# mathwrx/Decouple-and-Couple_Learning_in_Multi-Modal_Brain_Tumor_Segmentation

Hardware: AMD Instinct MI355X
Metric: training volumes/sec (4x128^3) (higher is better)
Workload: dtype bf16x3 forward (split-bf16 MFMA operands hi.hi+hi.lo+lo.hi: logits within 1e-3 of the fp32 reference) / bf16 data-gradient / bf16 weight-gradient MFMA operands; f32 accumulate, f32 storage, f32 master weights; 1 GPU; configs[1]: 1xMI355X, batch 2 per GPU, 4-modality 128^3 synthetic BraTS patches; fwd + softmax_dice + 4 sub-region/edge losses + bwd + Adam(amsgrad); random-init weights, dropout on; global_batch=2, parallelism=dp1, precision=bf16x3, dgrad_precision=bf16, wgrad_precision=bf16, mode=plan

## Files before the change

decouple-and-couple_learning_in_multi-modal_brain_tumor_segmentation_amd/csrc/gemm.hip:

```cpp
#include "common.h"
#include <cstdlib>

typedef struct cwf_gemm_args GemmArgs;


template <int TM, int TN, int GK>
__global__ __launch_bounds__(256) void gemm_mfma_kernel(const GemmArgs a) {
  constexpr int LDA_S = GK + 1, LDB_S = TN + 16;
  constexpr int IM = TM / 32, JN = TN / 32;
  constexpr int SA = TM * GK / 256, SB = TN * GK / 256;
  __shared__ float As[TM * LDA_S];
  __shared__ float Bs[GK * LDB_S];
  const int tid = threadIdx.x, lane = tid & 63, wave = tid >> 6;
  const int wr = wave >> 1, wc = wave & 1;
  const int r = lane & 15, kq = lane >> 4;
  const int zb = blockIdx.z / a.ZH, zh = blockIdx.z % a.ZH;
  const int m0 = blockIdx.y * TM, n0 = blockIdx.x * TN;
  const int64_t a_zoff = zb * a.sa_zb + zh * a.sa_zh;
  const float* A = ((a.A2 && n0 >= a.split_n) ? a.A2 : a.A) + a_zoff;
  const bool tabB = a.B_tab[0] != nullptr;
  const float* B = tabB ? a.B_tab[blockIdx.z] : a.B + zb * a.sb_zb + zh * a.sb_zh;
  if (a.B2 && m0 >= a.split_m) B = a.B2 + zb * a.sb_zb + zh * a.sb_zh;
  const bool a_drop = a.a_drop_p > 0.f;
  float* rowsum = a.rowsum_tab[0] ? a.rowsum_tab[blockIdx.z] : a.rowsum;
  const bool do_rs = rowsum != nullptr && blockIdx.x == 0 && wc == 0;

  f32x4 acc[IM][JN], accr[IM];
#pragma unroll
  for (int i = 0; i < IM; ++i) {
    accr[i] = (f32x4){0.f, 0.f, 0.f, 0.f};
#pragma unroll
    for (int j = 0; j < JN; ++j) acc[i][j] = (f32x4){0.f, 0.f, 0.f, 0.f};
  }

  const bool a_kfast = (a.sa_k == 1);
  const bool b_nfast = (a.sb_n == 1);
  int am[SA], ak[SA], bk[SB], bn[SB];
#pragma unroll
  for (int i = 0; i < SA; ++i) {
    if (a_kfast) { ak[i] = tid % GK; am[i] = tid / GK + (256 / GK) * i; } else { am[i] = tid % TM; ak[i] = tid / TM + (256 / TM) * i; }
  }
#pragma unroll
  for (int i = 0; i < SB; ++i) {
    if (b_nfast) { bn[i] = tid % TN; bk[i] = tid / TN + (256 / TN) * i; } else { bk[i] = tid % GK; bn[i] = tid / GK + (256 / GK) * i; }
  }
  float ra[SA], rb[SB];
  auto fetch = [&](int k0) {
#pragma unroll
    for (int i = 0; i < SA; ++i) {
      const int gm = m0 + am[i], gk = k0 + ak[i];
      float v = 0.f;
      if (gm < a.M && gk < a.K) {
        const int64_t off = gm * a.sa_m + gk * a.sa_k;
        v = A[off];
        if (a_drop) v *= cwf_keep(a.rng, a.a_drop_off, (uint64_t)(a_zoff + off), a.a_drop_n, a.a_drop_p, a.a_drop_p2);
      }
      ra[i] = v;
    }
#pragma unroll
    for (int i = 0; i < SB; ++i) {
      const int gn = n0 + bn[i], gkb = k0 + bk[i];
      rb[i] = (gn < a.N && gkb < a.K) ? B[gkb * a.sb_k + gn * a.sb_n] : 0.f;
    }
  };
  fetch(0);
  for (int k0 = 0; k0 < a.K; k0 += GK) {
    if (k0) __syncthreads();
#pragma unroll
    for (int i = 0; i < SA; ++i) As[am[i] * LDA_S + ak[i]] = ra[i];
#pragma unroll
    for (int i = 0; i < SB; ++i) Bs[bk[i] * LDB_S + bn[i]] = rb[i];
    __syncthreads();
    if (k0 + GK < a.K) fetch(k0 + GK);
#pragma unroll
    for (int kk = 0; kk < GK / 4; ++kk) {
      float av[IM], bv[JN];
#pragma unroll
      for (int i = 0; i < IM; ++i) av[i] = As[(wr * (TM / 2) + i * 16 + r) * LDA_S + kk * 4 + kq];
#pragma unroll
      for (int j = 0; j < JN; ++j) bv[j] = Bs[(kk * 4 + kq) * LDB_S + wc * (TN / 2) + j * 16 + r];
#pragma unroll
      for (int i = 0; i < IM; ++i)
#pragma unroll
        for (int j = 0; j < JN; ++j) acc[i][j] = __builtin_amdgcn_mfma_f32_16x16x4f32(av[i], bv[j], acc[i][j], 0, 0, 0);
      if (do_rs) {
#pragma unroll
        for (int i = 0; i < IM; ++i) accr[i] = __builtin_amdgcn_mfma_f32_16x16x4f32(av[i], 1.0f, accr[i], 0, 0, 0);
      }
    }
  }
  const int64_t c_zoff = zb * a.sc_zb + zh * a.sc_zh;
  float* C = a.C_tab[0] ? a.C_tab[blockIdx.z] : a.C + c_zoff;
  float* C2 = a.C2 ? a.C2 + c_zoff : nullptr;
  const float* bias = a.bias_tab[0] ? a.bias_tab[blockIdx.z] : a.bias;
  const float* R = a.residual ? a.residual + zb * a.sr_zb + zh * a.sr_zh : nullptr;
  const bool c_drop = a.c_drop_p > 0.f;
#pragma unroll
  for (int i = 0; i < IM; ++i)
#pragma unroll
    for (int j = 0; j < JN; ++j) {
      const int gn = n0 + wc * (TN / 2) + j * 16 + r;
      if (gn >= a.N) continue;
      const float bv = bias ? bias[gn] : 0.f;
#pragma unroll
      for (int e = 0; e < 4; ++e) {
        const int gm = m0 + wr * (TM / 2) + i * 16 + kq * 4 + e;
        if (gm >= a.M) continue;
        const int64_t off = gm * a.sc_m + gn;
        float v = acc[i][j][e] * a.alpha + bv;
        if (C2) C2[off] = v;
        if (a.act == 1) v = 0.5f * v * (1.f + erff(v * 0.70710678118654752440f));
        if (c_drop) v *= cwf_keep(a.rng, a.c_drop_off, (uint64_t)(c_zoff + off), a.c_drop_n, a.c_drop_p, a.c_drop_p2);
        if (R) v += R[gm * a.sr_m + gn];
        float* p = C + off;
        if (a.accumulate) v += *p;
        *p = v;
      }
    }
  if (do_rs && r == 0) {
#pragma unroll
    for (int i = 0; i < IM; ++i)
#pragma unroll
      for (int e = 0; e < 4; ++e) {
        const int gm = m0 + wr * (TM / 2) + i * 16 + kq * 4 + e;
        if (gm < a.M) rowsum[gm] = (a.rowsum_acc ? rowsum[gm] : 0.f) + accr[i][e];
      }
  }
}

template <int TM, int TN, int GK, bool AK, bool BN>
__global__ __launch_bounds__(256) void gemm_mfma_v_kernel(const GemmArgs a) {
  constexpr int LDA_S = GK + 1, LDB_S = TN + 16;
  constexpr int IM = TM / 32, JN = TN / 32;
  constexpr int SA = TM * GK / 1024, SB = TN * GK / 1024;
  __shared__ float As[TM * LDA_S];
  __shared__ __attribute__((aligned(16))) float Bs[GK * LDB_S];
  const int tid = threadIdx.x, lane = tid & 63, wave = tid >> 6;
  const int wr = wave >> 1, wc = wave & 1;
  const int r = lane & 15, kq = lane >> 4;
  const int zb = blockIdx.z / a.ZH, zh = blockIdx.z % a.ZH;
  const int m0 = blockIdx.y * TM, n0 = blockIdx.x * TN;
  const int64_t a_zoff = zb * a.sa_zb + zh * a.sa_zh;
  const float* A = ((a.A2 && n0 >= a.split_n) ? a.A2 : a.A) + a_zoff;
  const bool tabB = a.B_tab[0] != nullptr;
  const float* B = tabB ? a.B_tab[blockIdx.z] : a.B + zb * a.sb_zb + zh * a.sb_zh;
  if (a.B2 && m0 >= a.split_m) B = a.B2 + zb * a.sb_zb + zh * a.sb_zh;
  const bool a_drop = a.a_drop_p > 0.f;
  float* rowsum = a.rowsum_tab[0] ? a.rowsum_tab[blockIdx.z] : a.rowsum;
  const bool do_rs = rowsum != nullptr && blockIdx.x == 0 && wc == 0;

  f32x4 acc[IM][JN], accr[IM];
#pragma unroll
  for (int i = 0; i < IM; ++i) {
    accr[i] = (f32x4){0.f, 0.f, 0.f, 0.f};
#pragma unroll
    for (int j = 0; j < JN; ++j) acc[i][j] = (f32x4){0.f, 0.f, 0.f, 0.f};
  }
  int am[SA], ak[SA], bk[SB], bn[SB];
#pragma unroll
  for (int i = 0; i < SA; ++i) {
    if (AK) { ak[i] = (tid % (GK / 4)) * 4; am[i] = tid / (GK / 4) + (1024 / GK) * i; }
    else { am[i] = (tid % (TM / 4)) * 4; ak[i] = tid / (TM / 4) + (1024 / TM) * i; }
  }
#pragma unroll
  for (int i = 0; i < SB; ++i) {
    if (BN) { bn[i] = (tid % (TN / 4)) * 4; bk[i] = tid / (TN / 4) + (1024 / TN) * i; }
    else { bk[i] = (tid % (GK / 4)) * 4; bn[i] = tid / (GK / 4) + (1024 / GK) * i; }
  }
  f32x4 ra[SA], rb[SB];
  auto fetch = [&](int k0) {
#pragma unroll
    for (int i = 0; i < SA; ++i) {
      const int gm = m0 + am[i], gk = k0 + ak[i];
      f32x4 v = {0.f, 0.f, 0.f, 0.f};
      if (gm < a.M && gk < a.K) {
        const int64_t off = gm * a.sa_m + gk * a.sa_k;
        v = *reinterpret_cast<const f32x4*>(A + off);
        if (a_drop) {
          const int64_t st = AK ? 1 : a.sa_m;
#pragma unroll
          for (int c = 0; c < 4; ++c) v[c] *= cwf_keep(a.rng, a.a_drop_off, (uint64_t)(a_zoff + off + c * st), a.a_drop_n, a.a_drop_p, a.a_drop_p2);
        }
      }
      ra[i] = v;
    }
#pragma unroll
    for (int i = 0; i < SB; ++i) {
      const int gn = n0 + bn[i], gkb = k0 + bk[i];
      rb[i] = (gn < a.N && gkb < a.K) ? *reinterpret_cast<const f32x4*>(B + gkb * a.sb_k + gn * a.sb_n) : (f32x4){0.f, 0.f, 0.f, 0.f};
    }
  };
  fetch(0);
  for (int k0 = 0; k0 < a.K; k0 += GK) {
    if (k0) __syncthreads();
#pragma unroll
    for (int i = 0; i < SA; ++i)
#pragma unroll
      for (int c = 0; c < 4; ++c) {
        if (AK) As[am[i] * LDA_S + ak[i] + c] = ra[i][c];
        else As[(am[i] + c) * LDA_S + ak[i]] = ra[i][c];
      }
#pragma unroll
    for (int i = 0; i < SB; ++i) {
      if (BN) *reinterpret_cast<f32x4*>(&Bs[bk[i] * LDB_S + bn[i]]) = rb[i];
      else {
#pragma unroll
        for (int c = 0; c < 4; ++c) Bs[(bk[i] + c) * LDB_S + bn[i]] = rb[i][c];
      }
    }
    __syncthreads();
    if (k0 + GK < a.K) fetch(k0 + GK);
#pragma unroll
    for (int kk = 0; kk < GK / 4; ++kk) {
      float av[IM], bv[JN];
#pragma unroll
      for (int i = 0; i < IM; ++i) av[i] = As[(wr * (TM / 2) + i * 16 + r) * LDA_S + kk * 4 + kq];
#pragma unroll
      for (int j = 0; j < JN; ++j) bv[j] = Bs[(kk * 4 + kq) * LDB_S + wc * (TN / 2) + j * 16 + r];
#pragma unroll
      for (int i = 0; i < IM; ++i)
#pragma unroll
        for (int j = 0; j < JN; ++j) acc[i][j] = __builtin_amdgcn_mfma_f32_16x16x4f32(av[i], bv[j], acc[i][j], 0, 0, 0);
      if (do_rs) {
#pragma unroll
        for (int i = 0; i < IM; ++i) accr[i] = __builtin_amdgcn_mfma_f32_16x16x4f32(av[i], 1.0f, accr[i], 0, 0, 0);
      }
    }
  }
  const int64_t c_zoff = zb * a.sc_zb + zh * a.sc_zh;
  float* C = a.C_tab[0] ? a.C_tab[blockIdx.z] : a.C + c_zoff;
  float* C2 = a.C2 ? a.C2 + c_zoff : nullptr;
  const float* bias = a.bias_tab[0] ? a.bias_tab[blockIdx.z] : a.bias;
  const float* R = a.residual ? a.residual + zb * a.sr_zb + zh * a.sr_zh : nullptr;
  const bool c_drop = a.c_drop_p > 0.f;
#pragma unroll
  for (int i = 0; i < IM; ++i)
#pragma unroll
    for (int j = 0; j < JN; ++j) {
      const int gn = n0 + wc * (TN / 2) + j * 16 + r;
      if (gn >= a.N) continue;
      const float bv = bias ? bias[gn] : 0.f;
#pragma unroll
      for (int e = 0; e < 4; ++e) {
        const int gm = m0 + wr * (TM / 2) + i * 16 + kq * 4 + e;
        if (gm >= a.M) continue;
        const int64_t off = gm * a.sc_m + gn;
        float v = acc[i][j][e] * a.alpha + bv;
        if (C2) C2[off] = v;
        if (a.act == 1) v = 0.5f * v * (1.f + erff(v * 0.70710678118654752440f));
        if (c_drop) v *= cwf_keep(a.rng, a.c_drop_off, (uint64_t)(c_zoff + off), a.c_drop_n, a.c_drop_p, a.c_drop_p2);
        if (R) v += R[gm * a.sr_m + gn];
        float* p = C + off;
        if (a.accumulate) v += *p;
        *p = v;
      }
    }
  if (do_rs && r == 0) {
#pragma unroll
    for (int i = 0; i < IM; ++i)
#pragma unroll
      for (int e = 0; e < 4; ++e) {
        const int gm = m0 + wr * (TM / 2) + i * 16 + kq * 4 + e;
        if (gm < a.M) rowsum[gm] = (a.rowsum_acc ? rowsum[gm] : 0.f) + accr[i][e];
      }
  }
}

static bool gemm_vec_ok(const GemmArgs& a, bool* ak, bool* bn) {
  auto al = [](const void* p) { return (reinterpret_cast<uintptr_t>(p) & 15) == 0; };
  auto m4 = [](int64_t v) { return (v & 3) == 0; };
  if (!m4(a.sa_zb) || !m4(a.sa_zh) || !m4(a.sb_zb) || !m4(a.sb_zh)) return false;
  if (!al(a.A) || (a.A2 && !al(a.A2)) || (a.B && !al(a.B)) || (a.B2 && !al(a.B2))) return false;
  for (int z = 0; z < 4; ++z)
    if (a.B_tab[z] && !al(a.B_tab[z])) return false;
  if (a.sa_k == 1 && m4(a.K) && m4(a.sa_m)) *ak = true;
  else if (a.sa_m == 1 && m4(a.M) && m4(a.sa_k)) *ak = false;
  else return false;
  if (a.sb_n == 1 && m4(a.N) && m4(a.sb_k)) *bn = true;
  else if (a.sb_k == 1 && m4(a.K) && m4(a.sb_n)) *bn = false;
  else return false;
  if (a.B2 && (a.split_m & 3)) return false;
  return true;
}

struct GemmVariant { bool vec; int tm; bool ak, bn; };
static GemmVariant gemm_variant(const GemmArgs& a) {
  const int64_t wg64 = (int64_t)cdiv(a.N, 64) * cdiv(a.M, 64) * a.ZB * a.ZH;
  GemmVariant v = {false, wg64 >= 256 ? 64 : 32, false, false};
  if (a.K >= 64 && gemm_vec_ok(a, &v.ak, &v.bn)) v.vec = true;
  else v.ak = v.bn = false;
  return v;
}

static int gemm_check(const GemmArgs& a) {
  if (!a.A || (!a.B && !a.B_tab[0]) || (!a.C && !a.C_tab[0]) || a.M <= 0 || a.N <= 0 || a.K <= 0 || a.ZB <= 0 || a.ZH <= 0) return CWF_E_BADARG;
  if ((a.B_tab[0] || a.bias_tab[0] || a.C_tab[0] || a.rowsum_tab[0]) && (a.ZH != 1 || a.ZB > 4)) return CWF_E_BADARG;
  if ((int64_t)a.ZB * a.ZH > 65535) return CWF_E_TOOLARGE;
  if ((a.A2 && (a.split_n & 63)) || (a.B2 && (a.split_m & 63))) return CWF_E_BADARG;
  if ((a.a_drop_p > 0.f || a.c_drop_p > 0.f) && !a.rng) return CWF_E_BADARG;
  if (a.rowsum && (int64_t)a.ZB * a.ZH != 1) return CWF_E_BADARG;
  for (int z = 0; z < a.ZB && z < 4; ++z)
    if ((a.B_tab[0] && !a.B_tab[z]) || (a.bias_tab[0] && !a.bias_tab[z]) || (a.C_tab[0] && !a.C_tab[z]) || (a.rowsum_tab[0] && !a.rowsum_tab[z])) return CWF_E_BADARG;
  return 0;
}

extern "C" int cwf_gemm_ex(const struct cwf_gemm_args* args, void* stream) {
  if (!args) return CWF_E_BADARG;
  const GemmArgs& a = *args;
  const int rc = gemm_check(a);
  if (rc) return rc;
  const GemmVariant v = gemm_variant(a);
  const bool big = v.tm == 64;
  if (v.vec) {
    dim3 grid(cdiv(a.N, big ? 64 : 32), cdiv(a.M, big ? 64 : 32), a.ZB * a.ZH);
#define CWF_GV(AKv, BNv) do { if (big) hipLaunchKernelGGL((gemm_mfma_v_kernel<64, 64, 32, AKv, BNv>), grid, dim3(256), 0, cwf_stream(stream), a); \
                              else hipLaunchKernelGGL((gemm_mfma_v_kernel<32, 32, 64, AKv, BNv>), grid, dim3(256), 0, cwf_stream(stream), a); } while (0)
    if (v.ak && v.bn) CWF_GV(true, true); else if (v.ak) CWF_GV(true, false); else if (v.bn) CWF_GV(false, true); else CWF_GV(false, false);
#undef CWF_GV
    CWF_LAUNCH_CHECK();
    return 0;
  }
  if (big) {
    dim3 grid(cdiv(a.N, 64), cdiv(a.M, 64), a.ZB * a.ZH);
    hipLaunchKernelGGL((gemm_mfma_kernel<64, 64, 32>), grid, dim3(256), 0, cwf_stream(stream), a);
  } else {
    dim3 grid(cdiv(a.N, 32), cdiv(a.M, 32), a.ZB * a.ZH);
    hipLaunchKernelGGL((gemm_mfma_kernel<32, 32, 32>), grid, dim3(256), 0, cwf_stream(stream), a);
  }
  CWF_LAUNCH_CHECK();
  return 0;
}

extern "C" int cwf_debug_gemm_variant(const struct cwf_gemm_args* args, int* out) {
  if (!args || !out) return CWF_E_BADARG;
  const int rc = gemm_check(*args);
  if (rc) return rc;
  const GemmVariant v = gemm_variant(*args);
  out[0] = v.vec; out[1] = v.tm; out[2] = v.ak; out[3] = v.bn;
  return 0;
}

extern "C" int cwf_gemm(const float* A, int64_t sa_m, int64_t sa_k, int64_t sa_zb, int64_t sa_zh,
                        const float* B, int64_t sb_k, int64_t sb_n, int64_t sb_zb, int64_t sb_zh,
                        float* C, int64_t sc_m, int64_t sc_zb, int64_t sc_zh,
                        const float* bias, const float* residual, int64_t sr_m, int64_t sr_zb, int64_t sr_zh,
                        int M, int Nn, int K, int ZB, int ZH, float alpha, int act, int accumulate, void* stream) {
  GemmArgs a = {};
  a.A = A; a.sa_m = sa_m; a.sa_k = sa_k; a.sa_zb = sa_zb; a.sa_zh = sa_zh;
  a.B = B; a.sb_k = sb_k; a.sb_n = sb_n; a.sb_zb = sb_zb; a.sb_zh = sb_zh;
  a.C = C; a.sc_m = sc_m; a.sc_zb = sc_zb; a.sc_zh = sc_zh;
  a.bias = bias; a.residual = residual; a.sr_m = sr_m; a.sr_zb = sr_zb; a.sr_zh = sr_zh;
  a.M = M; a.N = Nn; a.K = K; a.ZB = ZB; a.ZH = ZH; a.alpha = alpha; a.act = act; a.accumulate = accumulate;
  return cwf_gemm_ex(&a, stream);
}

template <int PER>
__global__ __launch_bounds__(256) void layernorm_fwd_kernel(const float* __restrict__ x, const float* __restrict__ gamma, const float* __restrict__ beta,
                                                           float* __restrict__ y, float* __restrict__ mean, float* __restrict__ rstd, int rows, int E, float eps) {
  const int row = blockIdx.x * 4 + (threadIdx.x >> 6), lane = threadIdx.x & 63;
  if (row >= rows) return;
  const float* xr = x + (int64_t)row * E;
  float v[PER]; float s = 0.f;
#pragma unroll
  for (int i = 0; i < PER; ++i) { v[i] = xr[lane + 64 * i]; s += v[i]; }
  const float mu = wave_sum(s) / (float)E;
// ... 377 lines not shown
```

decouple-and-couple_learning_in_multi-modal_brain_tumor_segmentation_amd/cwf/_lib.py:

```python
from __future__ import annotations

import ctypes as C
import os

_HERE = os.path.dirname(os.path.abspath(__file__))
LIB_PATH = os.path.join(_HERE, "libcwf_hip.so")

P = C.c_void_p
I = C.c_int
L = C.c_int64
F = C.c_float
U = C.c_uint32
U64 = C.c_uint64
D = C.c_double

SIGNATURES = {
    "cwf_version": [],
    "cwf_conv": [P, P],
    "cwf_conv_x16_ok": [I, I, I, I, I, I, I],
    "cwf_debug_wsd": [I],
    "cwf_debug_wsd_launches": [],
    "cwf_wgrad": [P, P, P],
    "cwf_gather_split_bf16": [P, I, L, P],
    "cwf_wgrad_nsplit": [I, I, I, I, I, I, I],
    "cwf_wgrad_partial_floats": [I, I, I, I, I, I, I],
    "cwf_wgrad_slab_floats": [I, I, I],
    "cwf_wgrad_reduce": [P, I, L, P, P, P, P],
    "cwf_gather_batched": [P, I, L, P],
    "cwf_in_finalize": [P, P, P, I, L, F, P],
    "cwf_in_stats": [P, I, P, I, L, I, P],
    "cwf_norm_act_add": [P, I, P, P, F, P, I, P, I, I, L, I, P],
    "cwf_in_bwd_stats": [P, I, P, I, P, P, F, P, I, L, I, P],
    "cwf_in_bwd_apply": [P, I, P, I, P, P, F, P, P, I, P, I, I, L, I, P],
    "cwf_in_bwd_apply_ex": [P, I, P, I, P, P, F, P, P, I, P, I, P, P, I, L, I, P],
    "cwf_norm_act_add_ex": [P, I, P, P, F, P, I, P, I, P, I, L, I, P],
    "cwf_to_bf16": [P, I, P, P, F, P, I, L, I, P],
    "cwf_gemm": [P, L, L, L, L, P, L, L, L, L, P, L, L, L, P, P, L, L, L, I, I, I, I, I, F, I, I, P],
    "cwf_layernorm_fwd": [P, P, P, P, P, P, I, I, F, P],
    "cwf_layernorm_bwd": [P, P, P, P, P, P, P, P, I, I, I, P],
    "cwf_softmax_rows": [P, L, I, I, P],
    "cwf_softmax_rows_bwd": [P, P, L, I, I, P],
    "cwf_gelu_bwd": [P, P, P, L, P],
    "cwf_colsum": [P, L, I, I, P, I, P],
    "cwf_window_to_tokens": [P, I, P, I, I, I, I, I, I, I, I, P],
    "cwf_tokens_to_window": [P, P, I, I, I, I, I, I, I, I, I, I, P],
    "cwf_token_scores": [P, P, L, P, I, I, I, P],
    "cwf_topk": [P, P, I, I, I, P],
    "cwf_gather_tokens": [P, P, P, L, P, F, P, I, I, I, I, P],
    "cwf_gather_tokens_bwd": [P, P, P, P, P, L, I, I, I, I, P],
    "cwf_scatter_rows": [P, P, P, L, L, P, L, P, I, I, I, I, P],
    "cwf_scatter_rows_bwd": [P, P, P, P, L, P, I, P, L, L, P, L, I, I, I, I, P],
    "cwf_upsample_softmax": [P, I, P, I, I, I, I, I, I, P],
    "cwf_upsample_softmax_bwd": [P, P, P, I, I, I, I, I, I, I, P, P],
    "cwf_channel_softmax": [P, I, P, L, I, P],
    "cwf_channel_softmax_bwd": [P, P, P, I, L, I, P],
    "cwf_dice_ce_sums": [P, P, U, P, I, L, I, P],
    "cwf_dice_ce_finalize": [P, P, P, I, L, I, P],
    "cwf_dice_ce_bwd": [P, P, U, P, P, P, I, L, I, P],
    "cwf_adam_amsgrad": [P, I, L, C.c_double, C.c_double, C.c_double, C.c_double, C.c_double, I, I, P, P],
    "cwf_adam_amsgrad_scaled": [P, I, L, C.c_double, C.c_double, C.c_double, C.c_double, C.c_double, I, I, P, F, P],
    "cwf_grad_add": [P, P, P, L, P],
    "cwf_grad_norm_clip": [P, L, F, F, P, P, P],
    "cwf_adam_amsgrad_ex": [P, I, L, C.c_double, C.c_double, C.c_double, C.c_double, C.c_double, I, I, P, F, P, P, F, P],
    "cwf_optim_step": [I, P, I, L, C.c_double, C.c_double, P, C.c_double, C.c_double, C.c_double, I, I, P, C.c_double, C.c_double, I, I,
                       F, P, P, F, P],
    "cwf_wgrad_reduce_batched": [P, I, P],
    "cwf_dropout_mask": [P, L, F, F, C.c_uint64, C.c_uint64, P],
    "cwf_mul": [P, P, P, L, P],
    "cwf_add": [P, P, P, L, P],
    "cwf_channel_scale": [P, I, P, P, I, I, L, I, P],
    "cwf_copy_strided": [P, I, P, I, L, I, P],
    "cwf_add3": [P, P, P, P, L, P],
    "cwf_bcast3": [P, P, L, P],
    "cwf_stats_channel_sum": [P, P, I, I, P],
    "cwf_gemm_ex": [P, P],
    "cwf_attn_fwd": [P, L, P, L, I, I, I, I, F, P, U64, F, P],
    "cwf_attn_bwd": [P, L, P, L, P, I, I, I, I, F, P, U64, F, P],
    "cwf_ln_pair_fwd": [P, P, I, P, P, P, P, P, P, P, I, I, F, P],
    "cwf_ln_pair_bwd": [P, P, P, P, P, I, P, P, P, P, P, P, P, P, P, I, I, I, P],
    "cwf_gelu_bwd_drop": [P, P, P, L, P, U64, F, P],
    "cwf_token_scores2": [P, P, L, P, L, P, P, I, I, I, P],
    "cwf_topk_inv": [P, P, P, P, P, P, I, I, I, P],
    "cwf_index_inv": [P, P, I, I, I, P],
    "cwf_gather_multi": [P, I, I, I, I, F, P, F, P],
    "cwf_scatter_inv": [P, P, P, L, L, P, L, P, P, I, I, I, P],
    "cwf_scatter_bwd": [P, P, P, P, P, P, L, L, P, L, P, L, P, L, L, P, L, I, I, I, I, P],
    "cwf_token_grad": [P, P, P, L, P, P, P, L, P, L, P, U64, U64, F, P, I, I, I, I, P],
    "cwf_head_grad": [P, P, P, P, L, P, P, I, I, P],
    "cwf_dice_ce_finalize_multi": [P, P, P, P, I, I, L, I, P],
    "cwf_head_loss_sums": [P, I, I, P, P, P, I, I, I, I, I, P],
    "cwf_head_loss_bwd": [P, I, I, P, P, P, P, P, I, P, I, I, I, I, I, P],
    "cwf_head_loss_bwd_ex": [P, I, I, P, P, P, P, P, I, I, P, I, I, I, I, I, P],
    "cwf_ln_pair_fwd_g": [P, P, I, P, I, P, P, P, I, I, F, P],
    "cwf_ln_pair_bwd_g": [P, P, P, P, P, I, P, I, P, P, P, I, I, I, P],
    "cwf_token_scores2_g": [P, P, P, I, I, P, P, I, I, I, P],
    "cwf_head_grad_g": [P, P, P, P, L, P, P, I, I, I, P],
    "cwf_window_to_tokens_g": [P, I, P, I, I, I, I, I, I, I, I, I, P],
    "cwf_tokens_to_window_g": [P, P, I, I, I, I, I, I, I, I, I, I, P],
    "cwf_cat3_channels": [P, P, P, P, L, I, P],
    "cwf_stitch_windows": [P, P, I, P],
    "cwf_argmax_dice": [P, L, L, L, P, P, P, I, L, P],
    "cwf_argmax_metrics": [P, L, L, L, P, P, P, I, L, P],
    "cwf_region_bits": [P, P, L, P],
    "cwf_hausdorff_workspace": [I, I, I, I, I],
    "cwf_hausdorff": [P, P, I, I, I, I, I, D, D, D, I, I, P, P, P, P, L, P],
    "cwf_surface_metrics_workspace": [I, I, I, I, I],
    "cwf_surface_metrics": [P, P, I, I, I, I, I, D, D, D, I, I, P, I, P, P, P, P, P, P, P, P, L, P],
    "cwf_signed_distance_workspace": [I, I, I, I, I],
    "cwf_signed_distance": [P, P, P, I, I, I, I, I, P, P],
    "cwf_boundary_sums": [P, P, P, P, I, I, L, I, P],
    "cwf_boundary_finalize": [P, P, P, P, I, I, L, P],
    "cwf_boundary_bwd": [P, P, P, P, P, I, I, L, I, P],
    "cwf_topk_ce_workspace": [I, L],
    "cwf_topk_ce": [P, P, U, L, P, P, P, I, L, I, P, P],
    "cwf_topk_ce_bwd": [P, P, U, P, P, P, I, L, I, P],
    "cwf_focal_workspace": [I, L, I],
    "cwf_focal_loss": [P, P, P, I, P, P, P, P, I, L, I, P, P],
    "cwf_focal_loss_bwd": [P, P, P, I, P, P, P, P, I, L, I, P],
    "cwf_lovasz_workspace": [I, L, I],
    "cwf_lovasz": [P, P, P, I, I, P, P, P, P, I, L, P, P],
    "cwf_lovasz_bwd": [P, P, I, P, P, P, I, L, P],
    "cwf_components_workspace": [I, I, I, I, I],
    "cwf_components": [P, I, I, I, I, I, I, P, P, P, P, P, L, P],
    "cwf_postprocess_labels": [P, P, P, P, P, I, I, I, I, I, I, I, I, I, I, I, I, P, P, P],
    "cwf_label_metrics": [P, P, P, L, P],
    "cwf_dilate_bits": [P, P, I, I, I, I, I, I, P, L, P],
    "cwf_lesionwise_workspace": [I, I, I, I, I],
    "cwf_lesionwise": [P, P, I, I, I, I, I, I, L, D, P, P, P, P, P, P, L, P],
# ... 108 lines not shown


class PrepElasticSample(C.Structure):
    _fields_ = PrepAffineSample._fields_ + [("disp", P), ("G0", I), ("G1", I), ("G2", I)]


class IntensitySample(C.Structure):
    _fields_ = [("taps", (F * 7) * 4), ("amp", F * 4), ("key", U64), ("gamma", F * 4), ("blur", I), ("noise", I), ("gam", I)]


class FocalParams(C.Structure):
    _fields_ = [("fn", D), ("fp", D), ("exponent", D), ("smooth", D), ("gamma", D), ("ce_ratio", D), ("class_weight", D * 4)]


INTENSITY_TILE = (10, 10, 32)


def intensity_ws_floats(nb, crop):
    tiles = 1
    for c, t in zip(crop, INTENSITY_TILE):
        tiles *= (int(c) + t - 1) // t
    return 8 * int(nb) * tiles


class AcquireSample(C.Structure):
    _fields_ = [("bias", P * 4), ("G0", I), ("G1", I), ("G2", I), ("bias_mask", I), ("contrast_mask", I), ("lowres_mask", I),
                ("factor", F * 4), ("lattice", (I * 3) * 4)]


ACQUIRE_TILE = (32, 8, 32)


def acquire_ws_doubles(nb, crop):
    tiles = 1
    for c, t in zip(crop, ACQUIRE_TILE):
        tiles *= (int(c) + t - 1) // t
    return 12 * int(nb) * tiles


WINDOW_MAX_STARTS = 128


class WindowGrid(C.Structure):
    _fields_ = [("B", I), ("S", I * 3), ("r", I * 3), ("n", I * 3), ("start", (I * WINDOW_MAX_STARTS) * 3)]


class WindowBox(C.Structure):
    _fields_ = [("full", I * 3), ("lo", I * 3)]


NORM_WS_DOUBLES = 2568
GRADNORM_WS_DOUBLES = 1024
RULE_ADAMW, RULE_SGD = 1, 2
RESTYPE_INT64 = {"cwf_debug_wsd_launches", "cwf_wgrad_partial_floats", "cwf_wgrad_slab_floats", "cwf_hausdorff_workspace", "cwf_components_workspace",
                 "cwf_lesionwise_workspace", "cwf_surface_metrics_workspace", "cwf_lesionwise_ex_workspace", "cwf_signed_distance_workspace",
                 "cwf_topk_ce_workspace", "cwf_focal_workspace", "cwf_lovasz_workspace", "cwf_class_locations_workspace", "cwf_nonzero_box_workspace"}
LOCATIONS_TILE = 16384
NONZERO_BOX_TILE = 4096

_lib = None


class CwfError(RuntimeError):
    pass


def load():
    global _lib
    if _lib is not None:
        return _lib
    if not os.path.exists(LIB_PATH):
        raise CwfError("libcwf_hip.so is not built (%s); run `python __graft_entry__.py` or `make -C csrc`. "
                       "There is no CPU fallback." % LIB_PATH)
    lib = C.CDLL(LIB_PATH)
    for name, args in SIGNATURES.items():
        fn = getattr(lib, name)
        fn.argtypes = args
        fn.restype = L if name in RESTYPE_INT64 else I
    lib.cwf_arch.restype = C.c_char_p
    lib.cwf_arch.argtypes = []
    lib.cwf_plan_last_error.restype = C.c_char_p
    lib.cwf_plan_last_error.argtypes = []
    _lib = lib
    return lib


def check(rc, name):
    if rc != 0:
        raise CwfError("%s failed with status %d" % (name, rc))
```

include/cwf_hip.h:

```cpp
#ifndef CWF_HIP_H
#define CWF_HIP_H
#include <stdint.h>
#ifdef __cplusplus
extern "C" {
#endif

#define CWF_E_BADARG   (-1)
#define CWF_E_TOOLARGE (-2)
#define CWF_E_ALIGN    (-3)

int cwf_version(void);
const char* cwf_arch(void);

enum { CWF_CONV3_S1 = 0, CWF_CONV3_S2 = 1, CWF_CONV1 = 2, CWF_CONVT2 = 3, CWF_CONV3_S2_DGRAD = 4, CWF_CONVT2_DGRAD = 5 };
enum { CWF_FP32 = 0, CWF_BF16X3 = 1, CWF_BF16 = 2 };

struct cwf_conv_args {
  int op, precision;
  const float* x; int x_ldc; const void* wpk; const float* bias; float* y; int y_ldc;
  const float* in_scale; const float* in_shift; float in_slope;
  const float* residual; int r_ldc; const float* out_scale; double* stats;
  const float* nb_x; int nb_ldc; const float* nb_scale; const float* nb_shift; float nb_slope;
  const void* x16; const void* zero16; void* y16;
  const float* w_raw;
// ... 17 lines not shown
  int groups; const float* x_g[3]; const float* dy_g[3]; float* partial_g[3];
  int N, Di, Hi, Wi, Cin, Do, Ho, Wo, Cout;
};
int cwf_wgrad(const struct cwf_wgrad_args* args , int* nsplit_used , void* stream);
int cwf_wgrad_reduce(const float* partial, int nsplit, int64_t slab_floats,
                     const int32_t* inv_map, float* dW, float* db, void* stream);
struct cwf_wgrad_reduce_desc { const float* partial; const int32_t* inv; float* dW; float* db; int64_t slab; int32_t nsplit; int32_t pad_; };
int cwf_wgrad_reduce_batched(const struct cwf_wgrad_reduce_desc* table, int nlayers, void* stream);

struct cwf_gather_desc { const float* src; float* dst; const int32_t* map; int64_t n; };

int cwf_gather_split_bf16(const struct cwf_gather_desc* table, int nlayers, int64_t max_n, void* stream);

int cwf_gather_batched(const struct cwf_gather_desc* table, int nlayers, int64_t max_n, void* stream);

int cwf_in_finalize(const double* stats, float* scale, float* shift, int NC, int64_t V, float eps, void* stream);
int cwf_in_stats(const float* x, int x_ldc, double* stats, int N, int64_t V, int C, void* stream);
int cwf_norm_act_add(const float* x, int x_ldc, const float* scale, const float* shift, float slope,
                     const float* residual, int r_ldc, float* y, int y_ldc, int N, int64_t V, int C, void* stream);
int cwf_in_bwd_stats(const float* dy, int dy_ldc, const float* x, int x_ldc, const float* scale, const float* shift,
                     float slope, double* sums, int N, int64_t V, int C, void* stream);
int cwf_in_bwd_apply(const float* dy, int dy_ldc, const float* x, int x_ldc, const float* scale, const float* shift,
                     float slope, const double* sums, const float* dx_add, int a_ldc, float* dx, int dx_ldc,
                     int N, int64_t V, int C, void* stream);

int cwf_in_bwd_apply_ex(const float* dy, int dy_ldc, const float* x, int x_ldc, const float* scale, const float* shift,
                        float slope, const double* sums, const float* dx_add, int a_ldc, float* dx, int dx_ldc,
                        void* dx16, void* xa16, int N, int64_t V, int C, void* stream);
int cwf_norm_act_add_ex(const float* x, int x_ldc, const float* scale, const float* shift, float slope,
                        const float* residual, int r_ldc, float* y, int y_ldc, void* y16, int N, int64_t V, int C, void* stream);
int cwf_to_bf16(const float* x, int x_ldc, const float* scale, const float* shift, float slope, void* y16,
                int N, int64_t V, int C, void* stream);
int cwf_gemm(const float* A, int64_t sa_m, int64_t sa_k, int64_t sa_zb, int64_t sa_zh,
             const float* B, int64_t sb_k, int64_t sb_n, int64_t sb_zb, int64_t sb_zh,
             float* C, int64_t sc_m, int64_t sc_zb, int64_t sc_zh,
             const float* bias, const float* residual, int64_t sr_m, int64_t sr_zb, int64_t sr_zh,
             int M, int Nn, int K, int ZB, int ZH, float alpha, int act, int accumulate, void* stream);
struct cwf_gemm_args {
  const float* A; int64_t sa_m, sa_k, sa_zb, sa_zh;
  const float* B; int64_t sb_k, sb_n, sb_zb, sb_zh;
  float* C; int64_t sc_m, sc_zb, sc_zh;
  const float* bias; const float* residual; int64_t sr_m, sr_zb, sr_zh;
  int M, N, K, ZB, ZH; float alpha; int act; int accumulate;
  const float* A2; int split_n;
  const float* B2; int split_m;
  float* C2;
  float* rowsum; int rowsum_acc;
  const uint64_t* rng;
  uint64_t a_drop_off, a_drop_n; float a_drop_p, a_drop_p2;
  uint64_t c_drop_off, c_drop_n; float c_drop_p, c_drop_p2;
  const float* B_tab[4]; const float* bias_tab[4]; float* C_tab[4]; float* rowsum_tab[4];
};
int cwf_gemm_ex(const struct cwf_gemm_args* args , void* stream);

int cwf_attn_fwd(const float* qkv, int64_t ld, float* o, int64_t ldo, int Z, int T, int E, int heads, float scale,
                 const uint64_t* rng, uint64_t drop_off, float drop_p, void* stream);
int cwf_attn_bwd(const float* qkv, int64_t ld, const float* d_o, int64_t ldo, float* dqkv, int Z, int T, int E, int heads,
                 float scale, const uint64_t* rng, uint64_t drop_off, float drop_p, void* stream);

int cwf_ln_pair_fwd(const float* x, const float* x2, int perm_T, const float* g1, const float* b1, const float* g2, const float* b2,
                    float* ya, float* yb, float* stats, int rows, int E, float eps, void* stream);
struct cwf_ln_group_params { const float* g1[4]; const float* b1[4]; const float* g2[4]; const float* b2[4];
                             float* dg1[4]; float* db1[4]; float* dg2[4]; float* db2[4]; };
int cwf_ln_pair_fwd_g(const float* x, const float* x2, int perm_T, const struct cwf_ln_group_params* h_params, int groups,
                      float* ya, float* yb, float* stats, int rows, int E, float eps, void* stream);
int cwf_ln_pair_bwd_g(const float* dy, const float* da, const float* db, const float* x, const float* x2, int perm_T,
                      const struct cwf_ln_group_params* h_params, int groups, const float* stats, float* dx, float* dx2,
                      int rows, int E, int accumulate_params, void* stream);
int cwf_ln_pair_bwd(const float* dy, const float* da, const float* db, const float* x, const float* x2, int perm_T,
                    const float* g1, const float* g2, const float* stats, float* dx, float* dx2,
                    float* dg1, float* db1, float* dg2, float* db2, int rows, int E, int accumulate_params, void* stream);
int cwf_gelu_bwd_drop(const float* z, const float* dh, float* dz, int64_t n, const uint64_t* rng, uint64_t off, float p, void* stream);

int cwf_layernorm_fwd(const float* x, const float* gamma, const float* beta, float* y, float* mean, float* rstd,
                      int rows, int E, float eps, void* stream);
int cwf_layernorm_bwd(const float* dy, const float* x, const float* gamma, const float* mean, const float* rstd,
                      float* dx, float* dgamma, float* dbeta, int rows, int E, int accumulate, void* stream);
int cwf_softmax_rows(float* s, int64_t rows, int cols, int ld, void* stream);
int cwf_softmax_rows_bwd(const float* p, float* dp_inout, int64_t rows, int cols, int ld, void* stream);
int cwf_gelu_bwd(const float* x, const float* dy, float* dx, int64_t n, void* stream);
int cwf_colsum(const float* x, int64_t rows, int cols, int ld, float* out, int accumulate, void* stream);

int cwf_window_to_tokens(const float* x, int x_ldc, float* tok, int B, int D, int H, int W, int C,
                         int p0, int p1, int p2, void* stream);
int cwf_tokens_to_window(const float* tok, float* x, int x_ldc, int B, int D, int H, int W, int C,
                         int p0, int p1, int p2, int accumulate, void* stream);
int cwf_token_scores(const float* feats, const float* query, int64_t query_bstride, float* score,
                     int B, int T, int E, void* stream);
int cwf_topk(const float* score, int32_t* index, int B, int T, int k, void* stream);
int cwf_gather_tokens(const float* feats, const int32_t* index, const float* head, int64_t head_bstride,
                      const float* keep, float pe_odd, float* seq, int B, int T, int k, int E, void* stream);
int cwf_gather_tokens_bwd(const float* dseq, const int32_t* index, const float* keep, float* dfeats, float* dhead,
                          int64_t dhead_bstride, int B, int T, int k, int E, void* stream);
int cwf_scatter_rows(const float* feats, const int32_t* index, const float* rows, int64_t rows_ld, int64_t rows_bs,
                     const float* gate, int64_t gate_bs, float* out, int B, int T, int k, int E, void* stream);
int cwf_scatter_rows_bwd(const float* dout, const int32_t* index, const float* scat, const float* gate, int64_t gate_bs,
                         float* dfeats, int accumulate, float* drows, int64_t drows_ld, int64_t drows_bs,
                         float* dgate, int64_t dgate_bs, int B, int T, int k, int E, void* stream);

int cwf_token_scores2(const float* feats, const float* q1, int64_t q1_bstride, const float* q2, int64_t q2_bstride,
                      float* s1, float* s2, int B, int T, int E, void* stream);
int cwf_token_scores2_g(const float* feats, const float* const* h_q1, const float* const* h_q2, int groups, int group_B,
                        float* s1, float* s2, int B, int T, int E, void* stream);
int cwf_topk_inv(const float* score0, int32_t* index0, int32_t* inv0, const float* score1, int32_t* index1, int32_t* inv1,
                 int B, int T, int k, void* stream);
int cwf_index_inv(const int32_t* index, int32_t* inv, int B, int T, int k, void* stream);
// ... 262 lines not shown
```

Baseline: 117.9 volumes/s.

## Add compile-time-K panel GEMM kernel with deep register prefetch for common shapes

Adds a GEMM kernel specialised on a compile-time K. It prefetches several k-panels into registers ahead of use (depth D) and fully unrolls the panel loop. It also XOR-swizzles the shared-memory layout for the non-N-contiguous B operand. A routing table sends vectorisable GEMMs with matching K and tile size to this kernel by default, aiming to hide global-load latency and cut LDS bank conflicts in the transformer-path GEMMs. The shared epilogue is factored into a helper. The cost is more register pressure and code size from the deep prefetch and full unroll, plus extra template instantiations.

```diff
diff --git a/decouple-and-couple_learning_in_multi-modal_brain_tumor_segmentation_amd/csrc/gemm.hip b/decouple-and-couple_learning_in_multi-modal_brain_tumor_segmentation_amd/csrc/gemm.hip
--- a/decouple-and-couple_learning_in_multi-modal_brain_tumor_segmentation_amd/csrc/gemm.hip
+++ b/decouple-and-couple_learning_in_multi-modal_brain_tumor_segmentation_amd/csrc/gemm.hip
@@ -1,7 +1,51 @@
 #include "common.h"
 #include <cstdlib>
+#include <type_traits>
 
 typedef struct cwf_gemm_args GemmArgs;
+
+template <int TM, int TN>
+__device__ __forceinline__ void gemm_epilogue(const GemmArgs& a, const f32x4 (&acc)[TM / 32][TN / 32], const f32x4 (&accr)[TM / 32], int zb, int zh,
+                                              int m0, int n0, int wr, int wc, int r, int kq, bool do_rs, float* rowsum) {
+  constexpr int IM = TM / 32, JN = TN / 32;
+  const int64_t c_zoff = zb * a.sc_zb + zh * a.sc_zh;
+  float* C = a.C_tab[0] ? a.C_tab[blockIdx.z] : a.C + c_zoff;
+  float* C2 = a.C2 ? a.C2 + c_zoff : nullptr;
+  const float* bias = a.bias_tab[0] ? a.bias_tab[blockIdx.z] : a.bias;
+  const float* R = a.residual ? a.residual + zb * a.sr_zb + zh * a.sr_zh : nullptr;
+  const bool c_drop = a.c_drop_p > 0.f;
+#pragma unroll
+  for (int i = 0; i < IM; ++i)
+#pragma unroll
+    for (int j = 0; j < JN; ++j) {
+      const int gn = n0 + wc * (TN / 2) + j * 16 + r;
+      if (gn >= a.N) continue;
+      const float bv = bias ? bias[gn] : 0.f;
+#pragma unroll
+      for (int e = 0; e < 4; ++e) {
+        const int gm = m0 + wr * (TM / 2) + i * 16 + kq * 4 + e;
+        if (gm >= a.M) continue;
+        const int64_t off = gm * a.sc_m + gn;
+        float v = acc[i][j][e] * a.alpha + bv;
+        if (C2) C2[off] = v;
+        if (a.act == 1) v = 0.5f * v * (1.f + erff(v * 0.70710678118654752440f));
+        if (c_drop) v *= cwf_keep(a.rng, a.c_drop_off, (uint64_t)(c_zoff + off), a.c_drop_n, a.c_drop_p, a.c_drop_p2);
+        if (R) v += R[gm * a.sr_m + gn];
+        float* p = C + off;
+        if (a.accumulate) v += *p;
+        *p = v;
+      }
+    }
+  if (do_rs && r == 0) {
+#pragma unroll
+    for (int i = 0; i < IM; ++i)
+#pragma unroll
+      for (int e = 0; e < 4; ++e) {
+        const int gm = m0 + wr * (TM / 2) + i * 16 + kq * 4 + e;
+        if (gm < a.M) rowsum[gm] = (a.rowsum_acc ? rowsum[gm] : 0.f) + accr[i][e];
+      }
+  }
+}
 
 
 template <int TM, int TN, int GK>
@@ -89,43 +133,7 @@
       }
     }
   }
-  const int64_t c_zoff = zb * a.sc_zb + zh * a.sc_zh;
-  float* C = a.C_tab[0] ? a.C_tab[blockIdx.z] : a.C + c_zoff;
-  float* C2 = a.C2 ? a.C2 + c_zoff : nullptr;
-  const float* bias = a.bias_tab[0] ? a.bias_tab[blockIdx.z] : a.bias;
-  const float* R = a.residual ? a.residual + zb * a.sr_zb + zh * a.sr_zh : nullptr;
-  const bool c_drop = a.c_drop_p > 0.f;
-#pragma unroll
-  for (int i = 0; i < IM; ++i)
-#pragma unroll
-    for (int j = 0; j < JN; ++j) {
-      const int gn = n0 + wc * (TN / 2) + j * 16 + r;
-      if (gn >= a.N) continue;
-      const float bv = bias ? bias[gn] : 0.f;
-#pragma unroll
-      for (int e = 0; e < 4; ++e) {
-        const int gm = m0 + wr * (TM / 2) + i * 16 + kq * 4 + e;
-        if (gm >= a.M) continue;
-        const int64_t off = gm * a.sc_m + gn;
-        float v = acc[i][j][e] * a.alpha + bv;
-        if (C2) C2[off] = v;
-        if (a.act == 1) v = 0.5f * v * (1.f + erff(v * 0.70710678118654752440f));
-        if (c_drop) v *= cwf_keep(a.rng, a.c_drop_off, (uint64_t)(c_zoff + off), a.c_drop_n, a.c_drop_p, a.c_drop_p2);
-        if (R) v += R[gm * a.sr_m + gn];
-        float* p = C + off;
-        if (a.accumulate) v += *p;
-        *p = v;
-      }
-    }
-  if (do_rs && r == 0) {
-#pragma unroll
-    for (int i = 0; i < IM; ++i)
-#pragma unroll
-      for (int e = 0; e < 4; ++e) {
-        const int gm = m0 + wr * (TM / 2) + i * 16 + kq * 4 + e;
-        if (gm < a.M) rowsum[gm] = (a.rowsum_acc ? rowsum[gm] : 0.f) + accr[i][e];
-      }
-  }
+  gemm_epilogue<TM, TN>(a, acc, accr, zb, zh, m0, n0, wr, wc, r, kq, do_rs, rowsum);
 }
 
 template <int TM, int TN, int GK, bool AK, bool BN>
@@ -227,43 +235,149 @@
       }
     }
   }
-  const int64_t c_zoff = zb * a.sc_zb + zh * a.sc_zh;
-  float* C = a.C_tab[0] ? a.C_tab[blockIdx.z] : a.C + c_zoff;
-  float* C2 = a.C2 ? a.C2 + c_zoff : nullptr;
-  const float* bias = a.bias_tab[0] ? a.bias_tab[blockIdx.z] : a.bias;
-  const float* R = a.residual ? a.residual + zb * a.sr_zb + zh * a.sr_zh : nullptr;
-  const bool c_drop = a.c_drop_p > 0.f;
-#pragma unroll
-  for (int i = 0; i < IM; ++i)
-#pragma unroll
-    for (int j = 0; j < JN; ++j) {
-      const int gn = n0 + wc * (TN / 2) + j * 16 + r;
-      if (gn >= a.N) continue;
-      const float bv = bias ? bias[gn] : 0.f;
-#pragma unroll
-      for (int e = 0; e < 4; ++e) {
-        const int gm = m0 + wr * (TM / 2) + i * 16 + kq * 4 + e;
-        if (gm >= a.M) continue;
-        const int64_t off = gm * a.sc_m + gn;
-        float v = acc[i][j][e] * a.alpha + bv;
-        if (C2) C2[off] = v;
-        if (a.act == 1) v = 0.5f * v * (1.f + erff(v * 0.70710678118654752440f));
-        if (c_drop) v *= cwf_keep(a.rng, a.c_drop_off, (uint64_t)(c_zoff + off), a.c_drop_n, a.c_drop_p, a.c_drop_p2);
-        if (R) v += R[gm * a.sr_m + gn];
-        float* p = C + off;
-        if (a.accumulate) v += *p;
-        *p = v;
-      }
-    }
-  if (do_rs && r == 0) {
-#pragma unroll
-    for (int i = 0; i < IM; ++i)
-#pragma unroll
-      for (int e = 0; e < 4; ++e) {
-        const int gm = m0 + wr * (TM / 2) + i * 16 + kq * 4 + e;
-        if (gm < a.M) rowsum[gm] = (a.rowsum_acc ? rowsum[gm] : 0.f) + accr[i][e];
-      }
-  }
+  gemm_epilogue<TM, TN>(a, acc, accr, zb, zh, m0, n0, wr, wc, r, kq, do_rs, rowsum);
+}
+
+template <int TM, int TN, int PK, int KC, int D, bool AK, bool BN>
+__global__ __launch_bounds__(256) void gemm_mfma_p_kernel(const GemmArgs a) {
+  constexpr int NP = (KC + PK - 1) / PK;
+  constexpr int K4 = (KC + 3) / 4 * 4;
+  constexpr int LDA_S = PK + 1, LDB_S = TN + 16;
+  constexpr int IM = TM / 32, JN = TN / 32;
+  constexpr int SA = TM * PK / 1024, SB = TN * PK / 1024;
+  static_assert(D >= 2 && PK % 4 == 0 && SA >= 1 && SB >= 1, "panel geometry");
+  static_assert(KC % 4 == 0 || (!AK && BN), "an operand with 16-byte loads along k needs K % 4 == 0");
+  __shared__ float As[TM * LDA_S];
+  __shared__ __attribute__((aligned(16))) float Bs[PK * LDB_S];
+  const int tid = threadIdx.x, lane = tid & 63, wave = tid >> 6;
+  const int wr = wave >> 1, wc = wave & 1;
+  const int r = lane & 15, kq = lane >> 4;
+  const int zb = blockIdx.z / a.ZH, zh = blockIdx.z % a.ZH;
+  const int m0 = blockIdx.y * TM, n0 = blockIdx.x * TN;
+  const int64_t a_zoff = zb * a.sa_zb + zh * a.sa_zh;
+  const float* A = ((a.A2 && n0 >= a.split_n) ? a.A2 : a.A) + a_zoff;
+  const bool tabB = a.B_tab[0] != nullptr;
+  const float* B = tabB ? a.B_tab[blockIdx.z] : a.B + zb * a.sb_zb + zh * a.sb_zh;
+  if (a.B2 && m0 >= a.split_m) B = a.B2 + zb * a.sb_zb + zh * a.sb_zh;
+  const bool a_drop = a.a_drop_p > 0.f;
+  float* rowsum = a.rowsum_tab[0] ? a.rowsum_tab[blockIdx.z] : a.rowsum;
+  const bool do_rs = rowsum != nullptr && blockIdx.x == 0 && wc == 0;
+
+  f32x4 acc[IM][JN], accr[IM];
+#pragma unroll
+  for (int i = 0; i < IM; ++i) {
+    accr[i] = (f32x4){0.f, 0.f, 0.f, 0.f};
+#pragma unroll
+    for (int j = 0; j < JN; ++j) acc[i][j] = (f32x4){0.f, 0.f, 0.f, 0.f};
+  }
+  int am[SA], ak[SA], bk[SB], bn[SB];
+  int64_t aoff[SA], boff[SB];
+  bool a_ok[SA], b_ok[SB];
+  const int64_t a_sk = AK ? 1 : a.sa_k, a_sm = AK ? a.sa_m : 1, b_sn = BN ? 1 : a.sb_n, b_sk = BN ? a.sb_k : 1;
+#pragma unroll
+  for (int i = 0; i < SA; ++i) {
+    if (AK) { ak[i] = (tid % (PK / 4)) * 4; am[i] = tid / (PK / 4) + (1024 / PK) * i; }
+    else { am[i] = (tid % (TM / 4)) * 4; ak[i] = tid / (TM / 4) + (1024 / TM) * i; }
+    const int gm = m0 + am[i];
+    a_ok[i] = gm < a.M;
+    aoff[i] = min(gm, a.M - (AK ? 1 : 4)) * a_sm;
+  }
+#pragma unroll
+  for (int i = 0; i < SB; ++i) {
+    if (BN) { bn[i] = (tid % (TN / 4)) * 4; bk[i] = tid / (TN / 4) + (1024 / TN) * i; }
+    else { bk[i] = (tid % (PK / 4)) * 4; bn[i] = tid / (PK / 4) + (1024 / PK) * i; }
+    const int gn = n0 + bn[i];
+    b_ok[i] = gn < a.N;
+    boff[i] = min(gn, a.N - (BN ? 4 : 1)) * b_sn;
+  }
+  auto a_kmin = [](int i) { return AK ? 0 : (1024 / TM) * i; };
+  auto b_kmin = [](int i) { return BN ? (1024 / TN) * i : 0; };
+  f32x4 ra[D][SA], rb[D][SB];
+  auto fetch = [&](int p, f32x4 (&qa)[SA], f32x4 (&qb)[SB]) {
+    const int k0 = p * PK;
+    const bool tail = k0 + PK > KC;
+#pragma unroll
+    for (int i = 0; i < SA; ++i) {
+      if (k0 + a_kmin(i) >= K4) continue;
+      int gk = k0 + ak[i];
+      if (tail) gk = min(gk, KC - (AK ? 4 : 1));
+      qa[i] = *reinterpret_cast<const f32x4*>(A + aoff[i] + gk * a_sk);
+    }
+#pragma unroll
+    for (int i = 0; i < SB; ++i) {
+      if (k0 + b_kmin(i) >= K4) continue;
+      int gk = k0 + bk[i];
+      if (tail) gk = min(gk, KC - (BN ? 1 : 4));
+      qb[i] = *reinterpret_cast<const f32x4*>(B + boff[i] + gk * b_sk);
+    }
+  };
+  auto publish = [&](int p, const f32x4 (&qa)[SA], const f32x4 (&qb)[SB]) {
+    const int k0 = p * PK;
+    const bool tail = k0 + PK > KC;
+#pragma unroll
+    for (int i = 0; i < SA; ++i) {
+      if (k0 + a_kmin(i) >= K4) continue;
+      const int gk = k0 + ak[i];
+      const bool ok = a_ok[i] && (!tail || gk < KC);
+      f32x4 v = qa[i];
+      if (a_drop) {
+        const int64_t off = aoff[i] + (tail ? min(gk, KC - (AK ? 4 : 1)) : gk) * a_sk;
+#pragma unroll
+        for (int c = 0; c < 4; ++c) v[c] *= cwf_keep(a.rng, a.a_drop_off, (uint64_t)(a_zoff + off + c), a.a_drop_n, a.a_drop_p, a.a_drop_p2);
+      }
+#pragma unroll
+      for (int c = 0; c < 4; ++c) {
+        const float w = ok ? v[c] : 0.f;
+        if (AK) As[am[i] * LDA_S + ak[i] + c] = w;
+        else As[(am[i] + c) * LDA_S + ak[i]] = w;
+      }
+    }
+#pragma unroll
+    for (int i = 0; i < SB; ++i) {
+      if (k0 + b_kmin(i) >= K4) continue;
+      const bool ok = b_ok[i] && (!tail || k0 + bk[i] < KC);
+      f32x4 v = qb[i];
+#pragma unroll
+      for (int c = 0; c < 4; ++c) v[c] = ok ? v[c] : 0.f;
+      if (BN) *reinterpret_cast<f32x4*>(&Bs[bk[i] * LDB_S + bn[i]]) = v;
+      else {
+#pragma unroll
+        for (int c = 0; c < 4; ++c) Bs[(bk[i] + c) * LDB_S + (bn[i] ^ ((bk[i] >> 2) & 15))] = v[c];
+      }
+    }
+  };
+#pragma unroll
+  for (int p = 0; p < D && p < NP; ++p) fetch(p, ra[p], rb[p]);
+#pragma unroll
+  for (int p = 0; p < NP; ++p) {
+    if (p) __syncthreads();
+    publish(p, ra[p % D], rb[p % D]);
+    __syncthreads();
+    if (p + D < NP) fetch(p + D, ra[p % D], rb[p % D]);
+    constexpr int KK_ALL = PK / 4;
+    const int kk_n = (p + 1) * PK > K4 ? (K4 - p * PK) / 4 : KK_ALL;
+    auto mfmas = [&](auto rs) {
+#pragma unroll
+      for (int kk = 0; kk < KK_ALL; ++kk) {
+        if (kk >= kk_n) continue;
+        float av[IM], bv[JN];
+#pragma unroll
+        for (int i = 0; i < IM; ++i) av[i] = As[(wr * (TM / 2) + i * 16 + r) * LDA_S + kk * 4 + kq];
+#pragma unroll
+        for (int j = 0; j < JN; ++j) bv[j] = Bs[(kk * 4 + kq) * LDB_S + wc * (TN / 2) + j * 16 + (BN ? r : r ^ (kk & 15))];
+#pragma unroll
+        for (int i = 0; i < IM; ++i)
+#pragma unroll
+          for (int j = 0; j < JN; ++j) acc[i][j] = __builtin_amdgcn_mfma_f32_16x16x4f32(av[i], bv[j], acc[i][j], 0, 0, 0);
+        if (decltype(rs)::value) {
+#pragma unroll
+          for (int i = 0; i < IM; ++i) accr[i] = __builtin_amdgcn_mfma_f32_16x16x4f32(av[i], 1.0f, accr[i], 0, 0, 0);
+        }
+      }
+    };
+    if (do_rs) mfmas(std::true_type()); else mfmas(std::false_type());
+  }
+  gemm_epilogue<TM, TN>(a, acc, accr, zb, zh, m0, n0, wr, wc, r, kq, do_rs, rowsum);
 }
 
 static bool gemm_vec_ok(const GemmArgs& a, bool* ak, bool* bn) {
@@ -304,6 +418,32 @@
   return 0;
 }
 
+constexpr int GP_PK = 64, GP_D32 = 4, GP_PK64 = 32, GP_D64 = 4;
+typedef void (*GemmKernel)(const GemmArgs);
+struct GemmPanelEntry { bool ak, bn; int K, tm; bool product; GemmKernel kernel; };
+#define CWF_GP(AKv, BNv, Kv, TMv, PROD) {AKv, BNv, Kv, TMv, PROD, gemm_mfma_p_kernel<TMv, TMv, (TMv == 64 ? GP_PK64 : GP_PK), Kv, (TMv == 64 ? GP_D64 : GP_D32), AKv, BNv>}
+static const GemmPanelEntry g_gemm_panel_tab[] = {
+  CWF_GP(true, false, 512, 64, true),   CWF_GP(true, false, 512, 32, true),
+  CWF_GP(true, true, 512, 32, true),    CWF_GP(true, true, 1024, 32, true),
+  CWF_GP(false, true, 516, 64, true),   CWF_GP(false, true, 516, 32, true),   CWF_GP(false, true, 258, 32, true),
+  CWF_GP(true, false, GP_PK, 32, false), CWF_GP(true, false, GP_D32 * GP_PK, 32, false), CWF_GP(true, false, (GP_D32 + 1) * GP_PK, 32, false),
+  CWF_GP(true, true, GP_PK, 32, false),  CWF_GP(true, true, GP_D32 * GP_PK, 32, false),  CWF_GP(true, true, (GP_D32 + 1) * GP_PK, 32, false),
+  CWF_GP(false, true, GP_PK, 32, false), CWF_GP(false, true, GP_D32 * GP_PK, 32, false), CWF_GP(false, true, (GP_D32 + 1) * GP_PK, 32, false),
+};
+#undef CWF_GP
+
+static int g_gemm_panel = 1;
+static long long g_gemm_panel_launches = 0;
+extern "C" int cwf_debug_gemm_panel(int v) { const int old = g_gemm_panel; g_gemm_panel = v; return old; }
+extern "C" long long cwf_debug_gemm_panel_launches() { return g_gemm_panel_launches; }
+
+static const GemmPanelEntry* gemm_panel_route(const GemmArgs& a, const GemmVariant& v) {
+  if (!v.vec || g_gemm_panel == 0) return nullptr;
+  for (const GemmPanelEntry& e : g_gemm_panel_tab)
+    if (e.ak == v.ak && e.bn == v.bn && e.K == a.K && e.tm == v.tm) return (e.product || g_gemm_panel == 2) ? &e : nullptr;
+  return nullptr;
+}
+
 extern "C" int cwf_gemm_ex(const struct cwf_gemm_args* args, void* stream) {
   if (!args) return CWF_E_BADARG;
   const GemmArgs& a = *args;
@@ -311,6 +451,13 @@
   if (rc) return rc;
   const GemmVariant v = gemm_variant(a);
   const bool big = v.tm == 64;
+  if (const GemmPanelEntry* e = gemm_panel_route(a, v)) {
+    dim3 grid(cdiv(a.N, e->tm), cdiv(a.M, e->tm), a.ZB * a.ZH);
+    hipLaunchKernelGGL(e->kernel, grid, dim3(256), 0, cwf_stream(stream), a);
+    CWF_LAUNCH_CHECK();
+    ++g_gemm_panel_launches;
+    return 0;
+  }
   if (v.vec) {
     dim3 grid(cdiv(a.N, big ? 64 : 32), cdiv(a.M, big ? 64 : 32), a.ZB * a.ZH);
 #define CWF_GV(AKv, BNv) do { if (big) hipLaunchKernelGGL((gemm_mfma_v_kernel<64, 64, 32, AKv, BNv>), grid, dim3(256), 0, cwf_stream(stream), a); \
diff --git a/decouple-and-couple_learning_in_multi-modal_brain_tumor_segmentation_amd/cwf/_lib.py b/decouple-and-couple_learning_in_multi-modal_brain_tumor_segmentation_amd/cwf/_lib.py
--- a/decouple-and-couple_learning_in_multi-modal_brain_tumor_segmentation_amd/cwf/_lib.py
+++ b/decouple-and-couple_learning_in_multi-modal_brain_tumor_segmentation_amd/cwf/_lib.py
@@ -74,6 +74,8 @@
     "cwf_bcast3": [P, P, L, P],
     "cwf_stats_channel_sum": [P, P, I, I, P],
     "cwf_gemm_ex": [P, P],
+    "cwf_debug_gemm_panel": [I],
+    "cwf_debug_gemm_panel_launches": [],
     "cwf_attn_fwd": [P, L, P, L, I, I, I, I, F, P, U64, F, P],
     "cwf_attn_bwd": [P, L, P, L, P, I, I, I, I, F, P, U64, F, P],
     "cwf_ln_pair_fwd": [P, P, I, P, P, P, P, P, P, P, I, I, F, P],
@@ -288,7 +290,7 @@
 NORM_WS_DOUBLES = 2568
 GRADNORM_WS_DOUBLES = 1024
 RULE_ADAMW, RULE_SGD = 1, 2
-RESTYPE_INT64 = {"cwf_debug_wsd_launches", "cwf_wgrad_partial_floats", "cwf_wgrad_slab_floats", "cwf_hausdorff_workspace", "cwf_components_workspace",
+RESTYPE_INT64 = {"cwf_debug_wsd_launches", "cwf_debug_gemm_panel_launches", "cwf_wgrad_partial_floats", "cwf_wgrad_slab_floats", "cwf_hausdorff_workspace", "cwf_components_workspace",
                  "cwf_lesionwise_workspace", "cwf_surface_metrics_workspace", "cwf_lesionwise_ex_workspace", "cwf_signed_distance_workspace",
                  "cwf_topk_ce_workspace", "cwf_focal_workspace", "cwf_lovasz_workspace", "cwf_class_locations_workspace", "cwf_nonzero_box_workspace"}
 LOCATIONS_TILE = 16384
diff --git a/include/cwf_hip.h b/include/cwf_hip.h
--- a/include/cwf_hip.h
+++ b/include/cwf_hip.h
@@ -93,6 +93,8 @@
   const float* B_tab[4]; const float* bias_tab[4]; float* C_tab[4]; float* rowsum_tab[4];
 };
 int cwf_gemm_ex(const struct cwf_gemm_args* args , void* stream);
+int cwf_debug_gemm_panel(int v);
+long long cwf_debug_gemm_panel_launches(void);
 
 int cwf_attn_fwd(const float* qkv, int64_t ld, float* o, int64_t ldo, int Z, int T, int E, int heads, float scale,
                  const uint64_t* rng, uint64_t drop_off, float drop_p, void* stream);
```

Result: faster. 120.2 volumes/s (median of 6 runs) (+1.9%).
